# adobe-research/DiffusionHandles

Hardware: AMD Instinct MI355X
Metric: guided-denoise steps/sec at 512x512 (SD2-depth) (higher is better)
Workload: dtype f16

## Files before the change

### diffusionhandles_amd/csrc/gemm.hip

```cpp
#include <stdlib.h>

#include <vector>

#include <hip/hip_ext.h>

#include "gemm_k.h"

namespace dh {

struct GemmProf {
  bool on = false;
  std::vector<hipEvent_t> ev;
  size_t used = 0;
  double flops = 0;
  double bytes = 0;
  hipEvent_t e0 = nullptr, e1 = nullptr;
};
static GemmProf g_prof;
static int g_buf_stage = 1;
static int g_pp_force = 0;
struct GemmTileReport {
  int bm, bn, kg, stages, mw, splits, pp, gn_epi, reduce_gn;
};
static thread_local GemmTileReport g_last_tile;
// ... 246 lines not shown
      bs_w[j] = (unsigned)(((n >> 6) * KT) * 8192 + (n & 63) * 128);
    }
    if (MODE == GM_CONV_S1) {
      const int ky = tap / 3, kx = tap - ky * 3;
      bs_tap = (unsigned)((ky * p.Win + kx) * (int)p.lda + c0) * 2u;
      bs_sh = 31u - (unsigned)tap;
      bs_kx = kx;
      bs_step_px = (unsigned)((int)p.lda * 2);
      bs_step_row = (unsigned)((p.Win - 2) * (int)p.lda * 2);
    }
  }

  auto issue_piece = [&](int kt, int stage, int q) {
    const int k0 = kbeg + kt * BK;
    const unsigned sbase = __builtin_amdgcn_readfirstlane(lds0 + stage * STAGE + wave_s * 1024);
    if constexpr (BUF) {
      if (q < NPA) {
        const int j = q;
        const unsigned dst = sbase + (j * WG + grp) * (NWV * 1024);
        if (MODE == GM_DENSE) buf_dma16(bv_a[j], ra, (unsigned)k0 * 2u, dst);
        else buf_dma16(buf_mask_oob(bv_nt[j], bs_sh, bv_a[j]), ra, bs_tap, dst);
      } else {
        const int j = q - NPA;
        buf_dma16(bv_w, rw, bs_w[j] + (unsigned)(k0 >> 6) * 8192u, sbase + BM * 128 + (j * WG + grp) * (NWV * 1024));
      }
      return;
    }
    if (q < NPA) {
      const int j = q;
      if (MODE == GM_DENSE) {
        const T* ptr = Ag + a_off[j] + k0;
        dma16(ptr, sbase + (j * WG + grp) * (NWV * 1024));
      } else if (MODE == GM_CONV_S1) {
        const int ky = tap / 3, kx = tap - ky * 3;
        const long toff = ((long)(ky - 1) * p.Win + (kx - 1)) * p.lda + c0;
        const bool ok = (a_taps[j] & (1u << tap)) != 0;
        const T* ptr = Ag + a_off[j] + toff;
        dma16(ok ? ptr : zero, sbase + (j * WG + grp) * (NWV * 1024));
      } else {
        const int ky = tap / 3, kx = tap - ky * 3;
        bool ok = a_ok[j];
        int sy, sx;
        if (p.mode == A_CONV3) {
          const int iy = a_oy[j] * p.stride + ky - p.pad, ix = a_ox[j] * p.stride + kx - p.pad;
          ok = ok && iy >= 0 && ix >= 0 && iy < (p.Hin << p.up) && ix < (p.Win << p.up);
          sy = iy >> p.up; sx = ix >> p.up;
        } else {
          const int ty = a_oy[j] + ky - 1, tx = a_ox[j] + kx - 1;
          ok = ok && ty >= 0 && tx >= 0 && !(ty & 1) && !(tx & 1) && (ty >> 1) < p.Hin && (tx >> 1) < p.Win;
          sy = ty >> 1; sx = tx >> 1;
        }
        sy = sy < 0 ? 0 : (sy >= p.Hin ? p.Hin - 1 : sy);
        sx = sx < 0 ? 0 : (sx >= p.Win ? p.Win - 1 : sx);
        const T* ptr = Ag + (a_off[j] + (long)sy * p.Win + sx) * p.lda + c0 + lchunk * 8;
        dma16(ok ? ptr : zero, sbase + (j * WG + grp) * (NWV * 1024));
      }
    } else {
      const int j = q - NPA;
#ifdef DH_TUNING
      if (p.w_nt) dma16_nt(b_ptr[j] + (size_t)(k0 >> 6) * 4096, sbase + BM * 128 + (j * WG + grp) * (NWV * 1024));
      else
#endif
      dma16(b_ptr[j] + (size_t)(k0 >> 6) * 4096, sbase + BM * 128 + (j * WG + grp) * (NWV * 1024));
    }
  };
  auto next_tile = [&]() {
// ... 788 lines not shown
  g_last_tile.bm = BM; g_last_tile.bn = BN; g_last_tile.kg = KG; g_last_tile.stages = ST; g_last_tile.mw = MW;
  if (k.pp_a_bytes != 0 && gm != GM_GENERIC) launch_tile_b<T, BM, BN, ST, WG, KG, MW, true>(gm, lnf, grid, st, k, glu);
  else launch_tile_b<T, BM, BN, ST, WG, KG, MW, false>(gm, lnf, grid, st, k, glu);
}
#undef DH_GEMM_LAUNCH

#ifdef DH_TUNING
#define DH_KNOB(name, env, dflt) static const int name = getenv(env) ? atoi(getenv(env)) : (dflt)
#else
#define DH_KNOB(name, env, dflt) constexpr int name = (dflt)
#endif

template <class T>
static void gemm_dispatch(GemmK k, size_t partial_elems, hipStream_t st, int* gn_done, int* lnb_done, int dtype) {
  DH_KNOB(kSplitTiles, "DH_SPLITK_TILES", 200);
  DH_KNOB(kSplitMinK, "DH_SPLITK_MINKT", 32);
  DH_KNOB(kSplitTarget, "DH_SPLITK_TARGET", 256);
  DH_KNOB(kBigTiles, "DH_BIG_TILES", 128);
  DH_KNOB(kNarrowTiles, "DH_NARROW_TILES", 40);
  DH_KNOB(kN320, "DH_GEMM_N320", 224);
  DH_KNOB(kMwBlocks, "DH_GEMM_MW", 64);
  DH_KNOB(kKg2MinKt, "DH_KG2_MINKT", 4);
  DH_KNOB(kManyBlocks, "DH_GEMM_MANY", 512);
  DH_KNOB(kMw128, "DH_GEMM_MW128", 1);
  DH_KNOB(kTwoPerCu, "DH_GEMM_TWO_PER_CU", 1);
#ifdef DH_TUNING
  DH_KNOB(kWnt, "DH_W_NT", 0);
#endif
  const bool lnf = k.ln_s != nullptr;
  g_last_tile = GemmTileReport{};
  int BM = 128, BN = (k.N % 128 == 0) ? 128 : 64;
  const int ktiles = k.K / BK;
  PpPlan pp;
  const bool use_pp = gemm_pp_plan(k, partial_elems, g_pp_force, &pp);
  if (BN == 128 && ktiles >= 16 && cdiv(k.M, 128) * cdiv(k.N, 128) <= kNarrowTiles) BN = 64;
  if (k.M <= 64 || (cdiv(k.M, 128) * cdiv(k.N, BN) < kBigTiles && ktiles < kSplitMinK)) { BM = 64; BN = 64; }
  const bool n320 = kN320 > 0 && k.N % 320 == 0 && k.N <= 960 && !lnf && BM == 128 && BN == 64 && cdiv(k.M, 128) >= kN320;
  if (n320) BN = 320;
  DH_KNOB(kMwShortK, "DH_GEMM_MW_SHORTK", 128);
  const long tiles256 = (long)cdiv(k.M, 256) * cdiv(k.N, 128);
  const bool mw2 = kMwBlocks > 0 && k.N % 128 == 0 && tiles256 >= kMwBlocks &&
                   !(k.M <= 256 && k.M > 128 && cdiv(k.N, 128) < 128) && (tiles256 >= kMwShortK || ktiles >= kSplitMinK);
  if (mw2) { BM = 256; BN = 128; }
  const int glu = k.glu_y ? 1 : (k.glub_x ? 2 : 0);
  if (glu && !(BM == 64 && BN == 64)) { BM = mw2 ? 256 : 128; BN = 128; }
  DH_KNOB(kT160, "DH_GEMM_T160", 224);
  const long tiles160 = (long)cdiv(k.M, 128) * (k.N / 160);
  const bool t160 = kT160 > 0 && k.N % 160 == 0 && !lnf && !glu && !n320 && BM != 64 && tiles160 >= kT160 && tiles160 <= 256;
  if (t160) { BM = 128; BN = 160; }
  if (use_pp) { BM = pp.bm; BN = pp.bn; }
  const int tm = cdiv(k.M, BM), tn = cdiv(k.N, BN), tiles = tm * tn;
  int splits = 1;
  if (use_pp) splits = pp.splits;
  else if (k.partial && !lnf && !glu && tiles < kSplitTiles && ktiles >= kSplitMinK) {
    splits = kSplitTarget / tiles;
    if (splits > ktiles / 4) splits = ktiles / 4;
    if (splits > 32) splits = 32;
    const size_t fit = partial_elems / ((size_t)k.M * k.N);
    if ((size_t)splits > fit) splits = (int)fit;
    if (splits < 1) splits = 1;
  }
#ifdef DH_TUNING
  static const int kLog = getenv("DH_GEMM_LOG") ? atoi(getenv("DH_GEMM_LOG")) : 0;
  const int kForceTile = getenv("DH_FORCE_TILE") ? atoi(getenv("DH_FORCE_TILE")) : 0;
  const int kForceSplits = getenv("DH_FORCE_SPLITS") ? atoi(getenv("DH_FORCE_SPLITS")) : 0;
  int force_tile = 0;
  if (kForceTile && !use_pp && !(k.glu_y || k.glub_x)) {
// ... 38 lines not shown
#else
  dim3 grid(tm, tn, splits);
#endif
  hipEvent_t e0 = nullptr, e1 = nullptr;
  if (g_prof.on) {
    if (g_prof.used + 2 > g_prof.ev.size()) {
      const size_t old = g_prof.ev.size();
      g_prof.ev.resize(old + 4096);
      for (size_t i = old; i < g_prof.ev.size(); ++i) (void)hipEventCreate(&g_prof.ev[i]);
    }
    e0 = g_prof.ev[g_prof.used++];
    e1 = g_prof.ev[g_prof.used++];
    g_prof.flops += 2.0 * (double)k.M * (double)k.N * (double)k.K;
    const double esz = 2.0;
    double a_elems = (double)k.M * k.K;
    if (k.mode != A_DENSE && k.Hout > 0 && k.Wout > 0) a_elems = (double)k.M / ((double)k.Hout * k.Wout) * k.Hin * k.Win * k.Cin;
    double c_elems = (double)k.M * k.N * (k.C ? 1.0 : 0.0) + (k.R ? (double)k.M * k.N : 0.0);
    if (k.glu_y) c_elems += 0.5 * (double)k.M * k.N;
    if (k.glub_x) c_elems += 4.0 * (double)k.M * k.N;
    if (k.gn_epi == 2) c_elems += (double)k.M * k.N;
    g_prof.bytes += esz * (a_elems + (double)k.N * k.K + c_elems);
    g_prof.e0 = e0; g_prof.e1 = e1;
  }
  int gm = GM_GENERIC;
  if (k.mode == A_DENSE) gm = GM_DENSE;
  else if (k.mode == A_CONV3 && k.stride == 1 && k.up == 0 && k.pad == 1) gm = GM_CONV_S1;
  if (!use_pp) {
    k.pp_a_bytes = 0; k.pp_w_bytes = 0;
    size_t ab = 0;
    if (k.mode == A_DENSE) ab = ((size_t)(k.M - 1) * k.lda + k.K) * 2;
    else if (k.Hout > 0 && k.Wout > 0 && k.M % (k.Hout * k.Wout) == 0)
      ab = (size_t)(k.M / (k.Hout * k.Wout)) * k.Hin * k.Win * (size_t)k.lda * 2;
    const size_t wb = (size_t)align_up((size_t)k.N, 64) * k.K * 2;
    const bool conv_ok = k.mode == A_DENSE || (k.Cin % 64 == 0 && k.K == 9 * k.Cin);
    if ((g_buf_stage & 1) && ab > 0 && conv_ok && ab + (size_t)(k.Win + 1) * k.lda * 2 < 0x7ff00000ull && wb < 0x7ff00000ull && k.lda % 8 == 0 &&
        ((size_t)k.A & 15) == 0 && ((size_t)k.W & 15) == 0) {
      k.pp_a_bytes = (unsigned)ab; k.pp_w_bytes = (unsigned)wb;
    }
  }
#ifdef DH_TUNING
  static const int kAbl = getenv("DH_GEMM_ABLATE") ? atoi(getenv("DH_GEMM_ABLATE")) : 0;
  if (kAbl == 1 && BM == 128 && BN == 128) { hipLaunchKernelGGL((k_gemm_dma<T, 128, 128, 4, GM_CONV_S1, 1>), grid, dim3(256), 0, st, k); }
  else if (kAbl == 2 && BM == 128 && BN == 128) { hipLaunchKernelGGL((k_gemm_dma<T, 128, 128, 4, GM_CONV_S1, 2>), grid, dim3(256), 0, st, k); }
  else if (kAbl == 3 && BM == 128 && BN == 128) { hipLaunchKernelGGL((k_gemm_dma<T, 128, 128, 4, GM_DENSE, 1>), grid, dim3(256), 0, st, k); }
  else if (kAbl == 1 && mw2 && gm == GM_CONV_S1) { hipLaunchKernelGGL((k_gemm_dma<T, 256, 128, 3, GM_CONV_S1, 1, 1, 1, 2>), grid, dim3(512), 0, st, k); }
  else if (kAbl == 2 && mw2 && gm == GM_CONV_S1) { hipLaunchKernelGGL((k_gemm_dma<T, 256, 128, 3, GM_CONV_S1, 2, 1, 1, 2>), grid, dim3(512), 0, st, k); }
  else if (kAbl == 1 && mw2 && gm == GM_DENSE && !lnf) { hipLaunchKernelGGL((k_gemm_dma<T, 256, 128, 3, GM_DENSE, 1, 1, 1, 2>), grid, dim3(512), 0, st, k); }
  else if (kAbl == 2 && mw2 && gm == GM_DENSE && !lnf) { hipLaunchKernelGGL((k_gemm_dma<T, 256, 128, 3, GM_DENSE, 2, 1, 1, 2>), grid, dim3(512), 0, st, k); }
  else if (force_tile == 1) launch_tile<T, 64, 64, 4, 1, 1, 1>(gm, lnf, grid, st, k);
  else if (force_tile == 2) launch_tile<T, 128, 64, 3, 1, 2, 1>(gm, lnf, grid, st, k);
  else if (force_tile == 3) launch_tile<T, 128, 64, 5, 1, 1, 1>(gm, lnf, grid, st, k);
  else if (force_tile == 4) launch_tile<T, 128, 128, 4, 1, 1, 2>(gm, lnf, grid, st, k);
  else if (force_tile == 5) launch_tile<T, 128, 128, 4, 1, 1, 1>(gm, lnf, grid, st, k);
  else if (force_tile == 6) launch_tile<T, 256, 128, 3, 1, 1, 2>(gm, lnf, grid, st, k);
  else if (force_tile == 7) launch_tile<T, 128, 160, 4, 1, 1, 1>(gm, false, grid, st, k);
  else
#endif
  if (use_pp) { pp.splits = splits; g_last_tile.bm = pp.bm; g_last_tile.bn = pp.bn; launch_gemm_pp(dtype, k, pp, st, g_prof.e0, g_prof.e1); }
  else if (t160) launch_tile<T, 128, 160, 4, 1, 1, 1>(gm, false, grid, st, k);
  else if (mw2) launch_tile<T, 256, 128, 3, 1, 1, 2>(gm, lnf, grid, st, k, glu);
  else if (BM == 128 && BN == 128 && (glu || (kMw128 && tiles_per_split >= kMw128))) launch_tile<T, 128, 128, 4, 1, 1, 2>(gm, lnf, grid, st, k, glu);
  else if (kTwoPerCu && BM == 128 && BN == 64 && tiles * splits > 256 && tiles * splits <= 512)
    launch_tile<T, 128, 64, 3, 1, 1, 1>(gm, lnf, grid, st, k);
  else if (BM == 128 && BN == 64 && tiles_per_split >= kKg2MinKt) launch_tile<T, 128, 64, 3, 1, 2, 1>(gm, lnf, grid, st, k);
  else if (BN == 320) launch_tile<T, 128, 320, 2, 1, 1, 2>(gm, false, grid, st, k);
  else if (BM == 64) launch_tile<T, 64, 64, 4, 1, 1, 1>(gm, lnf, grid, st, k, glu);
  else if (BN == 128 && kManyBlocks > 0 && tiles * splits >= kManyBlocks) launch_tile<T, 128, 128, 2, 1, 1, 1>(gm, lnf, grid, st, k);
  else if (BN == 128) launch_tile<T, 128, 128, 4, 1, 1, 1>(gm, lnf, grid, st, k);
  else launch_tile<T, 128, 64, 5, 1, 1, 1>(gm, lnf, grid, st, k);
  g_prof.e0 = g_prof.e1 = nullptr;
  g_last_tile.splits = splits; g_last_tile.pp = use_pp ? 1 : 0; g_last_tile.gn_epi = k.gn_epi;
  if (k.gn_epi) *gn_done = k.gn_S;
  if (splits > 1) {
    if (k.gn_part && k.gn_G > 0 && k.gn_HW > 0 && k.N % k.gn_G == 0 && (GN_GB * (k.N / k.gn_G)) % 8 == 0 &&
        GN_GB * (k.N / k.gn_G) <= 2048 && k.M % k.gn_HW == 0) {
      k.gn_S = gn_slices(k.gn_HW, k.M / k.gn_HW);
      if (k.gnb_x) hipLaunchKernelGGL((k_splitk_reduce_gn<T, true>), dim3(k.gn_S, cdiv(k.gn_G, GN_GB), k.M / k.gn_HW), dim3(256), 0, st, k);
      else hipLaunchKernelGGL((k_splitk_reduce_gn<T, false>), dim3(k.gn_S, cdiv(k.gn_G, GN_GB), k.M / k.gn_HW), dim3(256), 0, st, k);
      g_last_tile.reduce_gn = 1;
      if (gn_done) *gn_done = 1;
    } else if (k.lnb_x && lnb_done && !k.bias && !k.rowvec && !k.R && !k.act_silu && k.N % 8 == 0 && k.ldc == k.N) {
      launch_splitk_reduce_ln_bwd(dtype, k.partial, splits, k.lnb_x, k.lnb_gamma, k.lnb_stats, k.lnb_add, k.lnb_dx, k.M, k.N, st);
      *lnb_done = 1;
    } else {
      const size_t groups = (size_t)k.M * k.N / 4;
      hipLaunchKernelGGL((k_splitk_reduce<T>), dim3((unsigned)((groups + 255) / 256)), dim3(256), 0, st, k);
    }
  }
}
#undef DH_KNOB

double launch_gemm(int dtype, const GemmArgs& a, hipStream_t st) {
  GemmK k;
  k.A = a.A; k.lda = a.lda; k.W = a.W; k.M = a.M; k.N = a.N; k.K = a.K;
  k.mode = a.mode; k.Hin = a.Hin; k.Win = a.Win; k.Cin = a.Cin; k.Hout = a.Hout; k.Wout = a.Wout;
  k.stride = a.stride; k.up = a.up; k.pad = a.pad;
  k.bias = a.bias; k.rowvec = a.rowvec; k.rowvec_ld = a.rowvec_ld;
  k.rows_per_batch = a.rows_per_batch > 0 ? a.rows_per_batch : 1;
  k.inv_rows_per_batch = 1.f / (float)k.rows_per_batch;
  k.R = a.R; k.ldr = a.ldr; k.C = a.C; k.ldc = a.ldc; k.act_silu = a.act_silu;
  k.partial = a.partial; k.splits = 1; k.k_per_split = a.K;
  k.pre_r = 1;
  k.wide_store = a.N % 32 == 0 && a.ldc % 8 == 0 && ((size_t)a.C & 15) == 0;
  k.ln_s = a.ln_s; k.ln_t = a.ln_t; k.ln_stats = a.ln_stats; k.ln_eps = a.ln_eps;
  k.gn_part = a.gn_part; k.gn_HW = a.gn_HW; k.gn_G = a.gn_G; k.gn_S = 0;
  k.gnb_x = a.gnb_x; k.gnb_ldx = a.gnb_ldx; k.gnb_gamma = a.gnb_gamma; k.gnb_beta = a.gnb_beta; k.gnb_stats = a.gnb_stats;
  k.gnb_silu = a.gnb_silu;
  k.lnb_x = a.lnb_x; k.lnb_gamma = a.lnb_gamma; k.lnb_stats = a.lnb_stats; k.lnb_add = a.lnb_add; k.lnb_dx = a.lnb_dx;
  k.glu_y = a.glu_y; k.glu_ldy = a.glu_ldy; k.glub_x = a.glub_x; k.glub_dx = a.glub_dx;
  if (a.gn_done) *a.gn_done = 0;
  if (a.lnb_done) *a.lnb_done = 0;
  if (dtype == DH_DTYPE_F16) gemm_dispatch<f16>(k, a.partial_elems, st, a.gn_done, a.lnb_done, dtype);
  else gemm_dispatch<bf16>(k, a.partial_elems, st, a.gn_done, a.lnb_done, dtype);
  return 2.0 * (double)a.M * (double)a.N * (double)a.K;
}

}

#ifdef DH_TUNING
extern "C" int dh_dbg_gemm_timeline(unsigned long long* ts) { dh::g_gemm_ts = ts; return DH_OK; }
#endif

extern "C" int dh_dbg_gemm_family(int force) {
  DH_REQUIRE(force >= 0 && force <= 2, "family: 0 policy, 1 k_gemm_dma, 2 k_gemm_pp");
  dh::g_pp_force = force;
  return DH_OK;
}

extern "C" int dh_dbg_gemm_stage(int buf) {
  dh::g_buf_stage = buf;
  return DH_OK;
}

extern "C" int dh_dbg_gemm_last_tile(int* out) {
  DH_REQUIRE(out != nullptr, "null pointer");
  const dh::GemmTileReport& r = dh::g_last_tile;
  const int v[9] = {r.bm, r.bn, r.kg, r.stages, r.mw, r.splits, r.pp, r.gn_epi, r.reduce_gn};
  for (int i = 0; i < 9; ++i) out[i] = v[i];
  return DH_OK;
}

extern "C" int dh_gemm_profile_begin(void) {
  dh::g_prof.on = true;
  dh::g_prof.used = 0;
// ... 24 lines not shown
```

### diffusionhandles_amd/csrc/gemm_k.h

```cpp
#pragma once
#include "unet_kernels.h"

namespace dh {

typedef _Float16 v8h __attribute__((ext_vector_type(8)));
typedef __bf16 v8b __attribute__((ext_vector_type(8)));
typedef float v16f __attribute__((ext_vector_type(16)));

template <class T> struct Mfma;
template <> struct Mfma<f16> {
  static __device__ __forceinline__ v16f run(uint4 a, uint4 b, v16f c) {
    return __builtin_amdgcn_mfma_f32_32x32x16_f16(__builtin_bit_cast(v8h, a), __builtin_bit_cast(v8h, b), c, 0, 0, 0);
  }
};
template <> struct Mfma<bf16> {
  static __device__ __forceinline__ v16f run(uint4 a, uint4 b, v16f c) {
    return __builtin_amdgcn_mfma_f32_32x32x16_bf16(__builtin_bit_cast(v8b, a), __builtin_bit_cast(v8b, b), c, 0, 0, 0);
  }
};

struct GemmK {
  const void* A; long lda;
  const void* W;
  int M, N, K;
  int mode, Hin, Win, Cin, Hout, Wout, stride, up, pad;
  const float* bias;
  const float* rowvec; int rowvec_ld; int rows_per_batch; float inv_rows_per_batch;
  const void* R; long ldr;
  void* C; long ldc;
  int act_silu;
  int pre_r;
  int wide_store;
#ifdef DH_TUNING
  int w_nt;
  unsigned long long* ts;
  int lnf_abl;
#endif
  const float* ln_s; const float* ln_t; float* ln_stats; float ln_eps;
  float* partial;
  int splits, k_per_split;
  float* gn_part; int gn_HW, gn_G, gn_S;
  int gn_epi, gn_cpg;
  const void* gnb_x; long gnb_ldx; const float *gnb_gamma, *gnb_beta, *gnb_stats; int gnb_silu;
  const void* lnb_x; const float *lnb_gamma, *lnb_stats; const void* lnb_add; void* lnb_dx;
  void* glu_y; long glu_ldy; const void* glub_x; void* glub_dx;
  int pp_tm, pp_tn, pp_order, pp_nwork; unsigned pp_a_bytes, pp_w_bytes;
  unsigned long long* pp_ts;
};


struct PpPlan { int bm = 0, bn = 0, splits = 1; };
bool gemm_pp_plan(const GemmK& k, size_t partial_elems, int force, PpPlan* plan);
void launch_gemm_pp(int dtype, const GemmK& k, const PpPlan& plan, hipStream_t st, hipEvent_t e0, hipEvent_t e1);

}
```

### diffusionhandles_amd/csrc/unet_engine.cpp

```cpp
#include <stdlib.h>

#include <algorithm>
#include <map>
#include <numeric>
#include <vector>

#include "unet_kernels.h"

namespace dh {

enum OpType { OP_CONV_IN, OP_CONV_OUT, OP_GEMM, OP_GN, OP_LN, OP_ATTN, OP_GEGLU, OP_CONCAT, OP_TIMESTEP, OP_T2F };
enum ParamKind { PK_F32, PK_MAT };

struct Ten {
  size_t off = 0, goff = 0;
  size_t off_fo = 0;
  int rows = 0, C = 0;
  bool req_grad = true;
  bool persistent = false;
};

struct Wt {
  size_t fwd_off = 0, bwd_off = 0;
  int N = 0, K = 0, taps = 1;
  bool has_bwd = true, f32 = false;
  int glu_F = 0;
};

struct ParamInfo {
  std::string name;
  int ndim = 0;
  int64_t shape[4] = {0, 0, 0, 0};
  int kind = PK_F32;
  size_t f32_off = 0;
  int wt = -1;
  int row_off = 0;
  int glu_F = 0;
};

struct Op {
  int type = OP_GEMM;
  int in0 = -1, in1 = -1, out = -1, res = -1;
  int wt = -1;
  long bias_off = -1;
  long gamma_off = -1, beta_off = -1;
  int mode = A_DENSE, Hin = 0, Win = 0, Cin = 0, Hout = 0, Wout = 0, stride = 1, up = 0;
  int in_col = 0, in_cols = 0;
  long rowvec_off = -1; int rowvec_ld = 0;
  int act_silu = 0;
  float eps = 1e-5f; int silu = 0; int groups = 32; size_t stats_off = 0;
  int heads = 0, Nq = 0, Nk = 0, cross = 0, kv_col = 0; size_t lse_off = 0;
  int gn_next = -1;
  int ln_fold = -1, folded = 0;
  long ln_s_off = -1, ln_t_off = -1;
  int glu_op = -1, glub_op = -1;
};

}

using namespace dh;

struct dh_unet {
  dh_unet_config cfg;
  int dtype = DH_DTYPE_F16;
  std::vector<Ten> tens;
  std::vector<Wt> wts;
  std::vector<ParamInfo> params;
  std::vector<Op> ops;
  std::map<std::string, int> pindex;
  size_t w16_elems = 0, pf_elems = 0, act_elems = 0, grad_elems = 0, f32_elems = 0;
  size_t fo_elems = 0;
  size_t partial_elems = 0, scratch_elems = 0, small_elems = 0;
  unsigned short *w16 = nullptr, *act = nullptr, *grad = nullptr, *scratch = nullptr;
  float *pf = nullptr, *f32a = nullptr, *partial = nullptr, *small = nullptr;
  int t_text = -1, t_kv = -1, t_conv_in_out = -1, t_final = -1, act_ids[3] = {-1, -1, -1};
  int act_op_end[3] = {0, 0, 0};
  int first_cross_op = 0;
  int saved_ops = 0;
  int temb_ops = 0, temb_rows = 0;
  float temb_t = 0.f;
  hipStream_t temb_stream = nullptr;
  uint64_t text_key = 0, kv_key = 0;
  int kv_rows = 0;
  hipStream_t kv_stream = nullptr;
  long temb_f32_off = -1;
  int temb_total = 0, kv_total = 0;
  float *in_sample = nullptr, *in_text = nullptr, *io_eps = nullptr, *out_dsample = nullptr, *out_dtext = nullptr, *t_dev = nullptr;
  std::map<uint64_t, hipGraphExec_t> graphs;
// ... 129 lines not shown
    Op o;
    o.type = OP_CONCAT; o.in0 = a; o.in1 = b;
    o.out = tensor(u.tens[a].rows, u.tens[a].C + u.tens[b].C);
    u.ops.push_back(o);
    return o.out;
  }

  void fold_ln_into_last_gemm() {
    const int gi = (int)u.ops.size() - 1, li = gi - 1;
    Op& g = u.ops[gi];
    Op& l = u.ops[li];
    if (g.type != OP_GEMM || l.type != OP_LN || g.in0 != l.out || g.mode != A_DENSE || g.in_col != 0) return;
    const int N = u.wts[g.wt].N;
    g.ln_fold = li; l.folded = 1;
    g.ln_s_off = (long)u.pf_elems; u.pf_elems += align_up((size_t)N, 64);
    g.ln_t_off = (long)u.pf_elems; u.pf_elems += align_up((size_t)N, 64);
  }

  int temb_cursor = 0, kv_cursor = 0;
  int wt_temb = -1, wt_kv = -1;
  size_t temb_bias_off = 0;

  int resnet(int x, const std::string& pre, int Cout, int H) {
    const int Cin = u.tens[x].C;
    int h = gn(x, pre + ".norm1", 1e-5f, true);
    bind_mat(pre + ".time_emb_proj.weight", wt_temb, Cout, temb_cursor, u.cfg.block_out_channels[0] * 4, 1);
    param_f32_at(pre + ".time_emb_proj.bias", Cout, temb_bias_off + temb_cursor);
    const long toff = temb_cursor;
    temb_cursor += Cout;
    h = conv3(h, pre + ".conv1", Cout, H, 1, 0, toff, -1);
    h = gn(h, pre + ".norm2", 1e-5f, true);
    int sc = x;
    if (Cin != Cout) sc = linear(x, pre + ".conv_shortcut", Cout, true, -1, true);
    return conv3(h, pre + ".conv2", Cout, H, 1, 0, -1, sc);
  }

  int transformer(int x, const std::string& pre, int heads, int H) {
    const int C = u.tens[x].C, N = H * H;
    int h = gn(x, pre + ".norm", 1e-6f, false);
    int t0 = linear(h, pre + ".proj_in", C, true, -1);
    const std::string b = pre + ".transformer_blocks.0";
    int n1 = ln(t0, b + ".norm1");
    const int wqkv = weight(3 * C, C);
    bind_mat(b + ".attn1.to_q.weight", wqkv, C, 0, C, 1);
    bind_mat(b + ".attn1.to_k.weight", wqkv, C, C, C, 1);
    bind_mat(b + ".attn1.to_v.weight", wqkv, C, 2 * C, C, 1);
    int qkv = linear_w(n1, wqkv, -1, -1);
    fold_ln_into_last_gemm();
    Op a;
    a.type = OP_ATTN; a.in0 = qkv; a.heads = heads; a.Nq = N; a.Nk = N; a.cross = 0;
    a.out = tensor(N, C);
    a.lse_off = f32_slot((size_t)maxB * heads * N);
    u.ops.push_back(a);
    int t1 = linear(a.out, b + ".attn1.to_out.0", C, true, t0);
    int n2 = ln(t1, b + ".norm2");
    int q2 = linear(n2, b + ".attn2.to_q", C, false, -1);
    fold_ln_into_last_gemm();
    bind_mat(b + ".attn2.to_k.weight", wt_kv, C, kv_cursor, u.cfg.cross_attention_dim, 1);
    bind_mat(b + ".attn2.to_v.weight", wt_kv, C, kv_cursor + C, u.cfg.cross_attention_dim, 1);
    Op c;
    c.type = OP_ATTN; c.in0 = q2; c.in1 = u.t_kv; c.heads = heads; c.Nq = N; c.Nk = u.cfg.text_len; c.cross = 1;
    c.kv_col = kv_cursor;
    kv_cursor += 2 * C;
    c.out = tensor(N, C);
    c.lse_off = f32_slot((size_t)maxB * heads * N);
    u.ops.push_back(c);
    int t2 = linear(c.out, b + ".attn2.to_out.0", C, true, t1);
// ... 129 lines not shown
  for (size_t i = 0; i + 1 < u.ops.size(); ++i) {
    Op& o = u.ops[i];
    const Op& nx = u.ops[i + 1];
    if (nx.type == OP_GN && nx.in0 == o.out && (o.type == OP_GEMM || o.type == OP_CONCAT)) o.gn_next = (int)(i + 1);
  }
  { int cmax = 0;
    for (const Op& o : u.ops) if (o.type == OP_LN) cmax = std::max(cmax, u.tens[o.in0].C);
    u.ones_off = (long)u.pf_elems; u.pf_elems += align_up((size_t)cmax, 64);
    u.zeros_off = (long)u.pf_elems; u.pf_elems += align_up((size_t)cmax, 64); }
  layout_tensors(u);
  size_t biggest = 0;
  for (const Ten& t : u.tens) biggest = std::max(biggest, (size_t)t.rows * t.C * c.max_diff_batch);
  u.scratch_elems = biggest * 4 + 1024;
  u.partial_elems = std::max<size_t>((size_t)48 << 20, biggest * 2);
  u.small_elems = (size_t)c.max_batch * 64 * 4096 + (size_t)c.max_batch * c.norm_groups * 4 + 4096;
  return DH_OK;
}


static void layout_tensors(dh_unet& u) {
  const size_t maxB = (size_t)u.cfg.max_batch, maxBd = (size_t)u.cfg.max_diff_batch;
  const int nt = (int)u.tens.size(), nops = (int)u.ops.size();
  u.tens[u.t_text].persistent = true;
  u.tens[u.t_kv].persistent = true;
  for (int i = 0; i < 3; ++i)
    if (u.act_ids[i] >= 0) u.tens[u.act_ids[i]].persistent = true;
  std::vector<int> first(nt, nops), last(nt, -1);
  auto rd = [&](int t, int oi) { if (t >= 0) { last[t] = std::max(last[t], oi); first[t] = std::min(first[t], oi); } };
  auto wr = [&](int t, int oi) { if (t >= 0) { first[t] = std::min(first[t], oi); last[t] = std::max(last[t], oi); } };
  for (int oi = 0; oi < nops; ++oi) {
    const Op& o = u.ops[oi];
    rd(o.in0, oi); rd(o.in1, oi); rd(o.res, oi); wr(o.out, oi);
    if (o.ln_fold >= 0) rd(u.ops[o.ln_fold].in0, oi);
    if (o.glu_op >= 0) wr(u.ops[o.glu_op].out, oi);
  }
  std::vector<char> written(nt, 0);
  for (const Op& o : u.ops) { if (o.out >= 0) written[o.out] = 1; if (o.glu_op >= 0) written[u.ops[o.glu_op].out] = 1; }
  for (int t = 0; t < nt; ++t)
    if (!written[t] || t == u.t_final) { first[t] = 0; last[t] = nops; u.tens[t].persistent = u.tens[t].persistent || !written[t]; }
  u.act_elems = 0; u.grad_elems = 0;
  for (Ten& t : u.tens) {
    t.off = u.act_elems;
    u.act_elems += align_up((size_t)t.rows * t.C * (t.persistent ? maxB : maxBd), 128);
    if (t.req_grad) { t.goff = u.grad_elems; u.grad_elems += align_up((size_t)t.rows * t.C * maxBd, 128); }
  }
  struct Live { size_t off, end; int last; };
  std::vector<Live> live;
  for (const Ten& t : u.tens)
    if (t.persistent) live.push_back({t.off, t.off + align_up((size_t)t.rows * t.C * maxB, 128), nops + 1});
  std::vector<int> order(nt);
  std::iota(order.begin(), order.end(), 0);
  std::stable_sort(order.begin(), order.end(), [&](int a, int b) { return first[a] < first[b]; });
  size_t fo_end = 0;
  for (const Live& l : live) fo_end = std::max(fo_end, l.end);
  for (int t : order) {
    Ten& tt = u.tens[t];
    if (tt.persistent) { tt.off_fo = tt.off; continue; }
    if (last[t] < 0) { tt.off_fo = 0; continue; }
    const size_t size = align_up((size_t)tt.rows * tt.C * maxB, 128);
    live.erase(std::remove_if(live.begin(), live.end(), [&](const Live& l) { return l.last < first[t]; }), live.end());
    std::sort(live.begin(), live.end(), [](const Live& a, const Live& b) { return a.off < b.off; });
    size_t pos = 0;
    for (const Live& l : live) {
      if (pos + size <= l.off) break;
      pos = std::max(pos, l.end);
    }
// ... 11 lines not shown
  const size_t idx = (size_t)blockIdx.x * blockDim.x + threadIdx.x;
  if (idx >= (size_t)N * C * taps) return;
  const int tap = (int)(idx % taps);
  const int cc = (int)((idx / taps) % C);
  int nn = (int)(idx / ((size_t)taps * C));
  if (glu_F) nn = glu_col(nn >= glu_F ? nn - glu_F : nn, nn >= glu_F ? 1 : 0);
  const D v = from_f32<D>(src[idx] * scale);
  int fk = tap * C + cc, bk = (taps - 1 - tap) * Nb + (int)col_off + nn;
  if (TILED && taps == 9) { fk = conv_k_index(tap, cc); bk = conv_k_index(taps - 1 - tap, (int)col_off + nn); }
  const int fr = (int)row_off + nn;
  if (TILED) {
    fwd[wt_index(fr, fk, (int)fwd_K)] = v;
    if (bwd) bwd[wt_index(cc, bk, (int)bwd_K)] = v;
  } else {
    fwd[(size_t)fr * fwd_K + fk] = v;
    if (bwd) bwd[(size_t)cc * bwd_K + bk] = v;
  }
}

}
namespace dh {
void launch_load_weight(int dtype, const float* src, int N, int C, int taps, void* fwd, long fwd_K, long row_off, void* bwd,
                        long bwd_K, long col_off, int Nb, float scale, hipStream_t st) {
  const size_t total = (size_t)N * C * taps;
  const unsigned nb = (unsigned)((total + 255) / 256);
  if (dtype == DH_DTYPE_F32)
    hipLaunchKernelGGL((k_load_weight<float, false>), dim3(nb), dim3(256), 0, st, src, N, C, taps, (float*)fwd, fwd_K, row_off, (float*)bwd, bwd_K, col_off, Nb, scale);
  else if (dtype == DH_DTYPE_F16)
    hipLaunchKernelGGL((k_load_weight<f16, true>), dim3(nb), dim3(256), 0, st, src, N, C, taps, (f16*)fwd, fwd_K, row_off, (f16*)bwd, bwd_K, col_off, Nb, scale);
  else
    hipLaunchKernelGGL((k_load_weight<bf16, true>), dim3(nb), dim3(256), 0, st, src, N, C, taps, (bf16*)fwd, fwd_K, row_off, (bf16*)bwd, bwd_K, col_off, Nb, scale);
}
}
namespace {

template <class D>
__global__ void __launch_bounds__(256) k_fold_ln(const D* bwd, int bwd_K, const float* gamma, const float* beta, const float* bias,
                                                 D* fwd, int K, float* s_out, float* t_out) {
  __shared__ float sm[8];
  const int n = blockIdx.x;
  float s = 0.f, t = 0.f;
  for (int k = threadIdx.x; k < K; k += blockDim.x) {
    const float w = to_f32<D>(bwd[wt_index(k, n, bwd_K)]);
    const D wf = from_f32<D>(w * gamma[k]);
    fwd[wt_index(n, k, K)] = wf;
    s += to_f32<D>(wf);
    t += beta[k] * w;
  }
  s = block_sum(s, sm);
  __syncthreads();
  t = block_sum(t, sm);
  if (threadIdx.x == 0) { s_out[n] = s; t_out[n] = t + (bias ? bias[n] : 0.f); }
}

__global__ void k_load_glu_bias(const float* src, float* dst, int F) {
  const int n = blockIdx.x * blockDim.x + threadIdx.x;
  if (n < 2 * F) dst[n] = src[glu_src_row(n, F)];
}

__global__ void k_fill_f32(float* p, int n, float v) {
  const int i = blockIdx.x * blockDim.x + threadIdx.x;
  if (i < n) p[i] = v;
}

static bool use_ln_fold(const dh_unet* u, int B) {
#ifdef DH_TUNING
  static const long lim = getenv("DH_LN_FOLD_MAXROWS") ? atol(getenv("DH_LN_FOLD_MAXROWS")) : 12288;
#else
  constexpr long lim = 12288;
#endif
  return (long)B * u->cfg.sample_size * u->cfg.sample_size <= lim;
}

static void fold_layernorms(dh_unet* u, hipStream_t st) {
  { int cmax = 0;
    for (const Op& o : u->ops) if (o.type == OP_LN) cmax = std::max(cmax, u->tens[o.in0].C);
    if (cmax > 0) {
      hipLaunchKernelGGL(k_fill_f32, dim3(cdiv(cmax, 256)), dim3(256), 0, st, u->pf + u->ones_off, cmax, 1.f);
      hipLaunchKernelGGL(k_fill_f32, dim3(cdiv(cmax, 256)), dim3(256), 0, st, u->pf + u->zeros_off, cmax, 0.f);
    } }
  for (const Op& g : u->ops) {
    if (g.type != OP_GEMM || g.ln_fold < 0) continue;
    const Op& l = u->ops[g.ln_fold];
    const Wt& w = u->wts[g.wt];
    const float* bias = g.bias_off >= 0 ? u->pf + g.bias_off : nullptr;
    if (u->dtype == DH_DTYPE_F16)
      hipLaunchKernelGGL((k_fold_ln<f16>), dim3(w.N), dim3(256), 0, st, (const f16*)(u->w16 + w.bwd_off), w.N, u->pf + l.gamma_off,
                         u->pf + l.beta_off, bias, (f16*)(u->w16 + w.fwd_off), w.K, u->pf + g.ln_s_off, u->pf + g.ln_t_off);
    else
      hipLaunchKernelGGL((k_fold_ln<bf16>), dim3(w.N), dim3(256), 0, st, (const bf16*)(u->w16 + w.bwd_off), w.N, u->pf + l.gamma_off,
                         u->pf + l.beta_off, bias, (bf16*)(u->w16 + w.fwd_off), w.K, u->pf + g.ln_s_off, u->pf + g.ln_t_off);
  }
  u->fold_dirty = false;
}

}

static int create_engine(const dh_unet_config* cfg, dh_unet* parent, dh_unet** out);
extern "C" int dh_unet_create(const dh_unet_config* cfg, dh_unet** out) {
  DH_REQUIRE(cfg && out, "null pointer");
  DH_REQUIRE(cfg->n_levels == 4, "n_levels must be 4");
  DH_REQUIRE(cfg->dtype == DH_DTYPE_F16 || cfg->dtype == DH_DTYPE_BF16, "dtype must be f16 or bf16");
  DH_REQUIRE(cfg->max_batch >= 1 && cfg->max_batch < 4096 && cfg->sample_size % 8 == 0 && cfg->sample_size >= 8, "bad batch / sample size");
  DH_REQUIRE((long)cfg->max_batch * cfg->sample_size * cfg->sample_size < (1L << 21), "max_batch * sample_size^2 must stay below 2^21 rows");
  DH_REQUIRE(cfg->norm_groups >= 1 && cfg->norm_groups <= 32, "1..32 GroupNorm groups");
  DH_REQUIRE(cfg->in_channels <= 8 && cfg->out_channels <= 8, "in/out channels must be <= 8");
  DH_REQUIRE(cfg->block_out_channels[0] <= 2048, "block_out_channels[0] must be <= 2048 (few-channel convolutions)");
  DH_REQUIRE(cfg->cross_attention_dim % 64 == 0, "cross_attention_dim must be a multiple of 64");
  for (int i = 0; i < 4; ++i) {
    DH_REQUIRE(cfg->block_out_channels[i] % 64 == 0, "block_out_channels must be multiples of 64");
    DH_REQUIRE(cfg->block_out_channels[i] == cfg->heads[i] * 64, "head dim must be 64");
    DH_REQUIRE(cfg->block_out_channels[i] % cfg->norm_groups == 0, "channels must divide into norm groups");
  }
  return create_engine(cfg, nullptr, out);
}

static int create_engine(const dh_unet_config* cfg, dh_unet* parent, dh_unet** out) {
  dh_unet* u = new dh_unet();
  u->cfg = *cfg;
  if (u->cfg.max_diff_batch <= 0 || u->cfg.max_diff_batch > u->cfg.max_batch) u->cfg.max_diff_batch = u->cfg.max_batch;
  u->dtype = cfg->dtype;
  int rc = build(*u);
  if (rc != DH_OK) { delete u; return rc; }
  auto fail = [&](hipError_t e, const char* what) {
    set_error(std::string(what) + ": " + hipGetErrorString(e));
    dh_unet_destroy(u);
// ... 156 lines not shown
}

static void forward_ops(dh_unet* u, int B, int n_ops, int first_op, bool kv_hit, bool save, hipStream_t st) {
  const int dt = u->dtype;
  const dh_unet_config& c = u->cfg;
  u->flops_fwd = 0;
  int gn_have = 0;
  if (!kv_hit) launch_f32_to_t(dt, u->in_text, u->aptr(u->t_text), (size_t)B * c.text_len * c.cross_attention_dim, st);
  for (int oi = first_op; oi < n_ops; ++oi) {
    const Op& o = u->ops[oi];
    if (kv_hit && oi == u->temb_ops) continue;
    switch (o.type) {
      case OP_TIMESTEP:
        launch_timestep_embedding(dt, u->t_dev, c.block_out_channels[0], B, u->aptr(o.out), st);
        break;
      case OP_T2F:
        launch_t_to_f32(dt, u->aptr(o.in0), u->f32a + u->temb_f32_off, (size_t)B * u->temb_total, 0, st);
        break;
      case OP_CONV_IN: {
        const Wt& w = u->wts[o.wt];
        launch_conv_small_fwd(dt, u->in_sample, 1, u->pf + w.fwd_off, u->pf + o.bias_off, u->aptr(o.out), 0, B, o.Hin, o.Hin,
                              o.Cin, w.N, st);
        u->flops_fwd += 2.0 * B * o.Hin * o.Hin * w.N * w.K;
        break;
      }
      case OP_CONV_OUT: {
        const Wt& w = u->wts[o.wt];
        launch_conv_small_fwd(dt, u->aptr(o.in0), 0, u->pf + w.fwd_off, u->pf + o.bias_off, u->io_eps, 1, B, o.Hin, o.Hin,
                              o.Cin, w.N, st);
        u->flops_fwd += 2.0 * B * o.Hin * o.Hin * w.N * w.K;
        break;
      }
      case OP_GEMM: {
        GemmArgs g;
        fill_gemm(u, o, B, g);
        gn_have = 0;
        if (o.gn_next >= 0 && oi + 1 < n_ops) {
          const Ten& to = u->tens[o.out];
          g.gn_part = u->small; g.gn_HW = to.rows; g.gn_G = u->ops[o.gn_next].groups; g.gn_done = &gn_have;
        }
        if (o.glu_op >= 0 && o.glu_op < n_ops) {
          const Op& ge = u->ops[o.glu_op];
          g.glu_y = u->aptr(ge.out); g.glu_ldy = u->tens[ge.out].C;
          if (!save) g.C = nullptr;
        }
        u->flops_fwd += launch_gemm(dt, g, st);
        break;
      }
      case OP_GN: {
        const Ten& t = u->tens[o.in0];
        const int have = (oi > 0 && u->ops[oi - 1].gn_next == oi) ? gn_have : 0;
        launch_groupnorm_fwd(dt, u->aptr(o.in0), u->pf + o.gamma_off, u->pf + o.beta_off, u->aptr(o.out),
                             u->f32a + o.stats_off, u->small, B, t.rows, t.C, o.groups, o.eps, o.silu, st, have);
        gn_have = 0;
        break;
      }
      case OP_LN: {
        if (o.folded && use_ln_fold(u, B)) break;
        const Ten& t = u->tens[o.in0];
        launch_layernorm_fwd(dt, u->aptr(o.in0), u->pf + (o.folded ? u->ones_off : o.gamma_off),
                             u->pf + (o.folded ? u->zeros_off : o.beta_off), u->aptr(o.out),
                             u->f32a + o.stats_off, B * t.rows, t.C, o.eps, st);
        break;
      }
      case OP_ATTN: {
        const Ten& tq = u->tens[o.in0];
        const int C = u->tens[o.out].C;
        if (!o.cross) {
// ... 441 lines not shown
```

### diffusionhandles_amd/csrc/unet_kernels.h

```cpp
#pragma once
#include "common.h"

namespace dh {

__device__ inline float silu_grad(float z) {
  const float s = 1.f / (1.f + __expf(-z));
  return s * (1.f + z * (1.f - s));
}

struct GeluParts { float Phi, pdf; };
__device__ __forceinline__ GeluParts gelu_parts(float g) {
  const float x = fabsf(g) * 0.70710678118654752f;
  const float t = __builtin_amdgcn_rcpf(fmaf(0.3275911f, x, 1.f));
  const float e = __expf(-x * x);
  const float poly = t * (0.254829592f + t * (-0.284496736f + t * (1.421413741f + t * (-1.453152027f + t * 1.061405429f))));
  const float q = 0.5f * poly * e;
  return {g < 0.f ? q : 1.f - q, e * 0.3989422804014327f};
}
__device__ __forceinline__ float gelu_f(float g) { return g * gelu_parts(g).Phi; }
__device__ __forceinline__ float gelu_grad(float g) { const GeluParts p = gelu_parts(g); return fmaf(g, p.pdf, p.Phi); }
__host__ __device__ inline int glu_col(int o, int gate) { return 32 * (o >> 4) + 16 * gate + (o & 15); }
__host__ __device__ inline int glu_src_row(int n, int F) { return ((n >> 4) & 1) * F + 16 * (n >> 5) + (n & 15); }

enum { A_DENSE = 0, A_CONV3 = 1, A_CONVT2 = 2 };

struct GemmArgs {
  const void* A = nullptr; long lda = 0;
  const void* W = nullptr;
  int M = 0, N = 0, K = 0;
  int mode = A_DENSE;
  int Hin = 0, Win = 0, Cin = 0;
  int Hout = 0, Wout = 0;
  int stride = 1, up = 0;
  int pad = 1;
  const float* bias = nullptr;
  const float* rowvec = nullptr; int rowvec_ld = 0; int rows_per_batch = 1;
  const void* R = nullptr; long ldr = 0;
  void* C = nullptr; long ldc = 0;
  int act_silu = 0;
  float* partial = nullptr; size_t partial_elems = 0;
  float* gn_part = nullptr; int gn_HW = 0, gn_G = 0; int* gn_done = nullptr;
  const void* gnb_x = nullptr; long gnb_ldx = 0; const float *gnb_gamma = nullptr, *gnb_beta = nullptr, *gnb_stats = nullptr;
  int gnb_silu = 0;
  const float* ln_s = nullptr; const float* ln_t = nullptr; float* ln_stats = nullptr; float ln_eps = 1e-5f;
  const void* lnb_x = nullptr; const float *lnb_gamma = nullptr, *lnb_stats = nullptr; const void* lnb_add = nullptr;
  void* lnb_dx = nullptr; int* lnb_done = nullptr;
  void* glu_y = nullptr; long glu_ldy = 0;
  const void* glub_x = nullptr; void* glub_dx = nullptr;
};
void launch_splitk_reduce_ln_bwd(int dtype, const float* partial, int splits, const void* x, const float* gamma,
                                 const float* stats, const void* add, void* dx, int rows, int C, hipStream_t st);
double launch_gemm(int dtype, const GemmArgs& a, hipStream_t st);
bool gemm_profiling_on();
void launch_tile_weights(int dtype, const void* src, void* dst, int N, int K, hipStream_t st, int conv_cin = 0);
__host__ __device__ inline size_t wt_index(int n, int k, int K) {
  const int r = n & 63, c = (k & 63) >> 3;
  return ((size_t)(n >> 6) * (K >> 6) + (k >> 6)) * 4096 + (size_t)r * 64 + (size_t)((c ^ ((r >> 1) & 7)) << 3) + (k & 7);
}

__host__ __device__ inline int conv_k_index(int tap, int c) { return (c >> 6) * 576 + tap * 64 + (c & 63); }

void launch_load_weight(int dtype, const float* src, int N, int C, int taps, void* fwd, long fwd_K, long row_off, void* bwd,
                        long bwd_K, long col_off, int Nb, float scale, hipStream_t st);

void launch_conv_small_fwd(int dtype, const void* x, int x_is_f32, const float* w, const float* bias, void* y,
                           int y_is_f32, int B, int H, int W, int Cin, int Cout, hipStream_t st);
void launch_conv_small_bwd(int dtype, const void* dy, int dy_is_f32, const float* w, void* dx, int dx_is_f32,
                           int accumulate, int B, int H, int W, int Cin, int Cout, hipStream_t st);

void launch_groupnorm_fwd(int dtype, const void* x, const float* gamma, const float* beta, void* y, float* stats,
                          float* scratch, int B, int HW, int C, int G, float eps, int silu, hipStream_t st,
                          int have_partials = 0);
int gn_slices(int HW, int B);
constexpr int GN_GB = 4;
void launch_concat_gn(int dtype, const void* a, int Ca, const void* b, int Cb, void* out, float* gn_part, int B, int HW,
                      int G, hipStream_t st);
struct GnBwdSplit { void* out0 = nullptr; void* out1 = nullptr; int split_c = 0; };
void launch_groupnorm_bwd(int dtype, const void* x, const void* dy, const float* gamma, const float* beta,
                          const float* stats, void* dx, float* scratch, int B, int HW, int C, int G, int silu,
                          int accumulate, hipStream_t st, int have_partials = 0, GnBwdSplit split = GnBwdSplit());
void launch_gelu(int dtype, const void* x, void* y, size_t n, hipStream_t st);
void launch_layernorm_fwd(int dtype, const void* x, const float* gamma, const float* beta, void* y, float* stats,
                          int rows, int C, float eps, hipStream_t st);
void launch_layernorm_bwd(int dtype, const void* x, const void* dy, const float* gamma, const float* stats,
                          const void* add, void* dx, int rows, int C, hipStream_t st);
// ... 28 lines not shown
```

Baseline: 35.60.

## Fold ResNet 1x1 shortcut GEMM into conv2 as extra K columns

When a ResNet block changes channel count, the 1x1 shortcut linear is now appended to the conv2 GEMM as a second A source. Its weights are concatenated along K and the two biases are summed, so one kernel replaces two. This drops a separate launch plus the write and re-read of the shortcut activation as a residual. Blocks that use the fused path give up the ping-pong and buffer-load paths, and the weights are folded at load time.

```diff
diff --git a/diffusionhandles_amd/csrc/gemm.hip b/diffusionhandles_amd/csrc/gemm.hip
--- a/diffusionhandles_amd/csrc/gemm.hip
+++ b/diffusionhandles_amd/csrc/gemm.hip
@@ -302,6 +302,12 @@
         const T* ptr = Ag + a_off[j] + k0;
         dma16(ptr, sbase + (j * WG + grp) * (NWV * 1024));
       } else if (MODE == GM_CONV_S1) {
+        if (k0 >= p.K1) {
+          const int m = m0 + 8 * (wave + NWV * (j * WG + grp)) + prow;
+          const T* ptr = reinterpret_cast<const T*>(p.A2) + (long)(m < p.M ? m : p.M - 1) * p.lda2 + lchunk * 8 + (k0 - p.K1);
+          dma16(ptr, sbase + (j * WG + grp) * (NWV * 1024));
+          return;
+        }
         const int ky = tap / 3, kx = tap - ky * 3;
         const long toff = ((long)(ky - 1) * p.Win + (kx - 1)) * p.lda + c0;
         const bool ok = (a_taps[j] & (1u << tap)) != 0;
@@ -1156,7 +1162,7 @@
   int BM = 128, BN = (k.N % 128 == 0) ? 128 : 64;
   const int ktiles = k.K / BK;
   PpPlan pp;
-  const bool use_pp = gemm_pp_plan(k, partial_elems, g_pp_force, &pp);
+  const bool use_pp = !k.A2 && gemm_pp_plan(k, partial_elems, g_pp_force, &pp);
   if (BN == 128 && ktiles >= 16 && cdiv(k.M, 128) * cdiv(k.N, 128) <= kNarrowTiles) BN = 64;
   if (k.M <= 64 || (cdiv(k.M, 128) * cdiv(k.N, BN) < kBigTiles && ktiles < kSplitMinK)) { BM = 64; BN = 64; }
   const bool n320 = kN320 > 0 && k.N % 320 == 0 && k.N <= 960 && !lnf && BM == 128 && BN == 64 && cdiv(k.M, 128) >= kN320;
@@ -1261,7 +1267,7 @@
     else if (k.Hout > 0 && k.Wout > 0 && k.M % (k.Hout * k.Wout) == 0)
       ab = (size_t)(k.M / (k.Hout * k.Wout)) * k.Hin * k.Win * (size_t)k.lda * 2;
     const size_t wb = (size_t)align_up((size_t)k.N, 64) * k.K * 2;
-    const bool conv_ok = k.mode == A_DENSE || (k.Cin % 64 == 0 && k.K == 9 * k.Cin);
+    const bool conv_ok = k.mode == A_DENSE || (k.Cin % 64 == 0 && k.K == 9 * k.Cin && !k.A2);
     if ((g_buf_stage & 1) && ab > 0 && conv_ok && ab + (size_t)(k.Win + 1) * k.lda * 2 < 0x7ff00000ull && wb < 0x7ff00000ull && k.lda % 8 == 0 &&
         ((size_t)k.A & 15) == 0 && ((size_t)k.W & 15) == 0) {
       k.pp_a_bytes = (unsigned)ab; k.pp_w_bytes = (unsigned)wb;
@@ -1319,9 +1325,10 @@
 }
 #undef DH_KNOB
 
-double launch_gemm(int dtype, const GemmArgs& a, hipStream_t st) {
+static GemmK gemm_k_of(const GemmArgs& a) {
   GemmK k;
   k.A = a.A; k.lda = a.lda; k.W = a.W; k.M = a.M; k.N = a.N; k.K = a.K;
+  k.A2 = a.K2 > 0 ? a.A2 : nullptr; k.lda2 = a.lda2; k.K1 = a.K - (a.K2 > 0 ? a.K2 : 0);
   k.mode = a.mode; k.Hin = a.Hin; k.Win = a.Win; k.Cin = a.Cin; k.Hout = a.Hout; k.Wout = a.Wout;
   k.stride = a.stride; k.up = a.up; k.pad = a.pad;
   k.bias = a.bias; k.rowvec = a.rowvec; k.rowvec_ld = a.rowvec_ld;
@@ -1337,8 +1344,24 @@
   k.gnb_silu = a.gnb_silu;
   k.lnb_x = a.lnb_x; k.lnb_gamma = a.lnb_gamma; k.lnb_stats = a.lnb_stats; k.lnb_add = a.lnb_add; k.lnb_dx = a.lnb_dx;
   k.glu_y = a.glu_y; k.glu_ldy = a.glu_ldy; k.glub_x = a.glub_x; k.glub_dx = a.glub_dx;
+  return k;
+}
+
+bool gemm_fold_shortcut(const GemmArgs& a) {
+  if (g_buf_stage & 16) return false;
+  PpPlan pp;
+  return !gemm_pp_plan(gemm_k_of(a), a.partial_elems, g_pp_force, &pp);
+}
+
+double launch_gemm(int dtype, const GemmArgs& a, hipStream_t st) {
+  GemmK k = gemm_k_of(a);
   if (a.gn_done) *a.gn_done = 0;
   if (a.lnb_done) *a.lnb_done = 0;
+  if (a.K2 > 0 && !(a.mode == A_CONV3 && a.stride == 1 && a.up == 0 && a.pad == 1 && a.K2 % 64 == 0 && a.K - a.K2 == 9 * a.Cin &&
+                    a.Cin % 64 == 0 && a.A2 && a.lda2 % 8 == 0)) {
+    fprintf(stderr, "launch_gemm: a second A source needs a stride-1 3x3 launch with whole 64-column K tiles\n");
+    abort();
+  }
   if (dtype == DH_DTYPE_F16) gemm_dispatch<f16>(k, a.partial_elems, st, a.gn_done, a.lnb_done, dtype);
   else gemm_dispatch<bf16>(k, a.partial_elems, st, a.gn_done, a.lnb_done, dtype);
   return 2.0 * (double)a.M * (double)a.N * (double)a.K;
diff --git a/diffusionhandles_amd/csrc/gemm_k.h b/diffusionhandles_amd/csrc/gemm_k.h
--- a/diffusionhandles_amd/csrc/gemm_k.h
+++ b/diffusionhandles_amd/csrc/gemm_k.h
@@ -23,6 +23,7 @@
   const void* A; long lda;
   const void* W;
   int M, N, K;
+  const void* A2; long lda2; int K1;
   int mode, Hin, Win, Cin, Hout, Wout, stride, up, pad;
   const float* bias;
   const float* rowvec; int rowvec_ld; int rows_per_batch; float inv_rows_per_batch;
diff --git a/diffusionhandles_amd/csrc/unet_engine.cpp b/diffusionhandles_amd/csrc/unet_engine.cpp
--- a/diffusionhandles_amd/csrc/unet_engine.cpp
+++ b/diffusionhandles_amd/csrc/unet_engine.cpp
@@ -54,6 +54,8 @@
   int ln_fold = -1, folded = 0;
   long ln_s_off = -1, ln_t_off = -1;
   int glu_op = -1, glub_op = -1;
+  int sc_op = -1, sc_wt = -1, sc_conv = -1;
+  long sc_bias_off = -1;
 };
 
 }
@@ -249,7 +251,20 @@
     h = gn(h, pre + ".norm2", 1e-5f, true);
     int sc = x;
     if (Cin != Cout) sc = linear(x, pre + ".conv_shortcut", Cout, true, -1, true);
-    return conv3(h, pre + ".conv2", Cout, H, 1, 0, -1, sc);
+    const int out = conv3(h, pre + ".conv2", Cout, H, 1, 0, -1, sc);
+    if (Cin != Cout) fold_shortcut_into_last_conv();
+    return out;
+  }
+  void fold_shortcut_into_last_conv() {
+    const int ci = (int)u.ops.size() - 1, si = ci - 1;
+    Op& c = u.ops[ci];
+    Op& s = u.ops[si];
+    if (c.mode != A_CONV3 || c.stride != 1 || c.up != 0 || s.type != OP_GEMM || s.mode != A_DENSE || c.res != s.out || s.in_col != 0) return;
+    const Wt w2 = u.wts[c.wt], ws = u.wts[s.wt];
+    if (w2.N != ws.N || w2.N % 64 != 0 || ws.K % 64 != 0 || w2.K != 9 * c.Cin || c.Cin % 64 != 0) return;
+    c.sc_op = si; s.sc_conv = ci;
+    c.sc_wt = weight(w2.N, w2.K + ws.K, 9, false);
+    c.sc_bias_off = (long)u.pf_elems; u.pf_elems += align_up((size_t)w2.N, 64);
   }
 
   int transformer(int x, const std::string& pre, int heads, int H) {
@@ -445,6 +460,7 @@
     const Op& o = u.ops[oi];
     rd(o.in0, oi); rd(o.in1, oi); rd(o.res, oi); wr(o.out, oi);
     if (o.ln_fold >= 0) rd(u.ops[o.ln_fold].in0, oi);
+    if (o.sc_op >= 0) rd(u.ops[o.sc_op].in0, oi);
     if (o.glu_op >= 0) wr(u.ops[o.glu_op].out, oi);
   }
   std::vector<char> written(nt, 0);
@@ -522,6 +538,7 @@
     hipLaunchKernelGGL((k_load_weight<bf16, true>), dim3(nb), dim3(256), 0, st, src, N, C, taps, (bf16*)fwd, fwd_K, row_off, (bf16*)bwd, bwd_K, col_off, Nb, scale);
 }
 }
+static void fill_gemm(dh_unet* u, const Op& o, int B, GemmArgs& g);
 namespace {
 
 template <class D>
@@ -560,6 +577,11 @@
   constexpr long lim = 12288;
 #endif
   return (long)B * u->cfg.sample_size * u->cfg.sample_size <= lim;
+}
+
+__global__ void k_add_f32(const float* a, const float* b, float* out, int n) {
+  const int i = blockIdx.x * blockDim.x + threadIdx.x;
+  if (i < n) out[i] = a[i] + b[i];
 }
 
 static void fold_layernorms(dh_unet* u, hipStream_t st) {
@@ -581,7 +603,26 @@
       hipLaunchKernelGGL((k_fold_ln<bf16>), dim3(w.N), dim3(256), 0, st, (const bf16*)(u->w16 + w.bwd_off), w.N, u->pf + l.gamma_off,
                          u->pf + l.beta_off, bias, (bf16*)(u->w16 + w.fwd_off), w.K, u->pf + g.ln_s_off, u->pf + g.ln_t_off);
   }
+  for (const Op& c : u->ops) {
+    if (c.type != OP_GEMM || c.sc_op < 0) continue;
+    const Op& sc = u->ops[c.sc_op];
+    const Wt &w2 = u->wts[c.wt], &ws = u->wts[sc.wt], &wf = u->wts[c.sc_wt];
+    const size_t tile = 64 * 64 * 2, rows = (size_t)(w2.N / 64);
+    unsigned short* dst = u->w16 + wf.fwd_off;
+    (void)hipMemcpy2DAsync(dst, (size_t)(wf.K / 64) * tile, u->w16 + w2.fwd_off, (size_t)(w2.K / 64) * tile, (size_t)(w2.K / 64) * tile,
+                           rows, hipMemcpyDeviceToDevice, st);
+    (void)hipMemcpy2DAsync(dst + (size_t)(w2.K / 64) * 4096, (size_t)(wf.K / 64) * tile, u->w16 + ws.fwd_off, (size_t)(ws.K / 64) * tile,
+                           (size_t)(ws.K / 64) * tile, rows, hipMemcpyDeviceToDevice, st);
+    hipLaunchKernelGGL(k_add_f32, dim3(cdiv(w2.N, 256)), dim3(256), 0, st, u->pf + c.bias_off, u->pf + sc.bias_off, u->pf + c.sc_bias_off, w2.N);
+  }
   u->fold_dirty = false;
+}
+
+static bool shortcut_folded(dh_unet* u, const Op& c, int B) {
+  if (c.sc_op < 0) return false;
+  GemmArgs g;
+  fill_gemm(u, c, B, g);
+  return gemm_fold_shortcut(g);
 }
 
 }
@@ -804,8 +845,17 @@
         break;
       }
       case OP_GEMM: {
+        if (o.sc_conv >= 0 && shortcut_folded(u, u->ops[o.sc_conv], B)) break;
         GemmArgs g;
         fill_gemm(u, o, B, g);
+        if (shortcut_folded(u, o, B)) {
+          const Op& sc = u->ops[o.sc_op];
+          const Wt& wf = u->wts[o.sc_wt];
+          g.W = u->w16 + wf.fwd_off; g.K = wf.K; g.K2 = u->wts[sc.wt].K;
+          g.A2 = u->aptr(sc.in0); g.lda2 = u->tens[sc.in0].C;
+          g.bias = u->pf + o.sc_bias_off;
+          g.R = nullptr; g.ldr = 0;
+        }
         gn_have = 0;
         if (o.gn_next >= 0 && oi + 1 < n_ops) {
           const Ten& to = u->tens[o.out];
diff --git a/diffusionhandles_amd/csrc/unet_kernels.h b/diffusionhandles_amd/csrc/unet_kernels.h
--- a/diffusionhandles_amd/csrc/unet_kernels.h
+++ b/diffusionhandles_amd/csrc/unet_kernels.h
@@ -28,6 +28,7 @@
   const void* A = nullptr; long lda = 0;
   const void* W = nullptr;
   int M = 0, N = 0, K = 0;
+  const void* A2 = nullptr; long lda2 = 0; int K2 = 0;
   int mode = A_DENSE;
   int Hin = 0, Win = 0, Cin = 0;
   int Hout = 0, Wout = 0;
@@ -51,6 +52,7 @@
 void launch_splitk_reduce_ln_bwd(int dtype, const float* partial, int splits, const void* x, const float* gamma,
                                  const float* stats, const void* add, void* dx, int rows, int C, hipStream_t st);
 double launch_gemm(int dtype, const GemmArgs& a, hipStream_t st);
+bool gemm_fold_shortcut(const GemmArgs& a);
 bool gemm_profiling_on();
 void launch_tile_weights(int dtype, const void* src, void* dst, int N, int K, hipStream_t st, int conv_cin = 0);
 __host__ __device__ inline size_t wt_index(int n, int k, int K) {
```

After: 35.93, median of 6. No clear change (+0.9%).
